# Hi-PACE/hipace

Measured on AMD Instinct MI355X. Metric: transverse slices/s at 1024^2 x 4ppc (explicit solver), higher is better.
Workload: dtype f64

## Files before the change

### hipace_amd/_lib.py

```python
import ctypes as C
import os
import subprocess


def hip_already_started():
    import sys
    if _LIB is not None:
        return True
    t = sys.modules.get("torch")
    try:
        return bool(t is not None and t.cuda.is_initialized())
    except Exception:
        return False


_LIB = None
_HWQ_PRESET = "GPU_MAX_HW_QUEUES" in os.environ
_HIP_STARTED_AT_IMPORT = hip_already_started()
_HERE = os.path.dirname(os.path.abspath(__file__))
CSRC = os.path.join(_HERE, "csrc")
SO = os.environ.get("HPS_LIB") or os.path.join(CSRC, "libhpslice.so")


class Slab(C.Structure):
# ... 115 lines not shown
                                           C.c_int, C.c_int, C.c_void_p, C.c_void_p, C.c_void_p]),
    "hps_deposit_current_tiled_laser": (C.c_int, [Slab, Plasma, Geom, C.c_void_p, C.c_int, C.c_double, C.c_double, C.c_int,
                                                  C.c_double, C.c_int, C.c_void_p, C.c_void_p, C.c_void_p, C.c_void_p]),
    "hps_explicit_deposit_tiled_laser": (C.c_int, [Slab, Plasma, Geom, C.c_void_p, C.c_int, C.c_void_p, C.c_double, C.c_double,
                                                   C.c_int, C.c_int, C.c_int, C.c_void_p, C.c_void_p, C.c_void_p]),
    "hps_advance_plasma_tiled_laser": (C.c_int, [Slab, Plasma, Geom, C.c_void_p, C.c_int, C.c_double, C.c_double, C.c_int,
                                                 C.c_int, C.c_int, C.c_int, C.c_void_p, C.c_void_p, C.c_void_p]),
    "hps_tiling_set_validity": (C.c_int, [C.c_void_p, C.c_int, C.c_int]),
    "hps_particles_record": (C.c_int, [C.c_int]),
    "hps_particles_recorded": (C.c_int, [C.c_char_p, C.c_long, C.POINTER(C.c_long)]),
    "hps_poisson_create": (C.c_int, [C.c_int, C.c_int, C.c_double, C.c_double, C.POINTER(C.c_void_p)]),
    "hps_poisson_solve": (C.c_int, [C.c_void_p, C.c_void_p, Slab, C.c_int, C.c_void_p]),
    "hps_poisson_solve_batch": (C.c_int, [C.c_void_p, C.c_int, C.c_void_p, Slab, C.c_void_p, C.c_void_p]),
    "hps_poisson_info": (C.c_int, [C.c_void_p, C.POINTER(C.c_int), C.POINTER(C.c_int), C.POINTER(C.c_int)]),
    "hps_poisson_destroy": (C.c_int, [C.c_void_p]),
    "hps_mg_create": (C.c_int, [C.c_int, C.c_int, C.c_double, C.c_double, C.POINTER(C.c_void_p)]),
    "hps_mg_solve1": (C.c_int, [C.c_void_p, Slab, C.c_int, C.c_int, C.c_int, C.c_double, C.c_double, C.c_int,
                                C.POINTER(C.c_int), C.POINTER(C.c_double), C.c_void_p]),
    "hps_mg_solve1_fabs": (C.c_int, [C.c_void_p, Slab, Slab, Slab, C.c_double, C.c_double, C.c_int,
                                     C.POINTER(C.c_int), C.POINTER(C.c_double), C.c_void_p]),
    "hps_mg_info": (C.c_int, [C.c_void_p, C.POINTER(C.c_int), C.POINTER(C.c_int), C.POINTER(C.c_int), C.POINTER(C.c_int),
                              C.POINTER(C.c_long), C.POINTER(C.c_int), C.POINTER(C.c_int), C.POINTER(C.c_int), C.POINTER(C.c_int)]),
    "hps_mg_info_schedule": (C.c_int, [C.c_void_p, C.POINTER(C.c_int)]),
    "hps_mg_destroy": (C.c_int, [C.c_void_p]),
    "hps_mg2_create": (C.c_int, [C.c_int, C.c_int, C.c_double, C.c_double, C.POINTER(C.c_void_p)]),
    "hps_mg2_solve2": (C.c_int, [C.c_void_p, C.c_void_p, C.c_void_p, C.c_void_p, C.c_void_p, C.c_double, C.c_double, C.c_int,
                                 C.POINTER(C.c_int), C.POINTER(C.c_double), C.c_void_p]),
    "hps_mg2_info": (C.c_int, [C.c_void_p, C.POINTER(C.c_int), C.POINTER(C.c_int), C.POINTER(C.c_int), C.POINTER(C.c_int)]),
    "hps_mg2_destroy": (C.c_int, [C.c_void_p]),
    "hps_engine_laser_vcycles": (C.c_int, [C.c_void_p, C.POINTER(C.c_long)]),
    "hps_engine_create": (C.c_int, [C.POINTER(Deck), C.c_int, C.POINTER(C.c_void_p)]),
    "hps_engine_destroy": (C.c_int, [C.c_void_p]),
    "hps_engine_begin_step": (C.c_int, [C.c_void_p]),
    "hps_engine_solve_slice": (C.c_int, [C.c_void_p, C.c_int]),
    "hps_engine_solve_slice_begin": (C.c_int, [C.c_void_p, C.c_int]),
    "hps_engine_solve_slice_finish": (C.c_int, [C.c_void_p, C.c_int]),
    "hps_engine_slice_ready": (C.c_int, [C.c_void_p]),
    "hps_engine_run_step": (C.c_int, [C.c_void_p]),
    "hps_engine_sync": (C.c_int, [C.c_void_p]),
    "hps_engine_info": (C.c_int, [C.c_void_p, C.POINTER(C.c_int), C.POINTER(C.c_int), C.POINTER(C.c_long)]),
    "hps_engine_slab": (Slab, [C.c_void_p]),
    "hps_engine_plasma": (Plasma, [C.c_void_p]),
    "hps_engine_stream": (C.c_void_p, [C.c_void_p]),
    "hps_engine_ions": (Plasma, [C.c_void_p]),
    "hps_engine_ion_stats": (C.c_int, [C.c_void_p, C.POINTER(C.c_long), C.POINTER(C.c_long)]),
    "hps_engine_checksums": (C.c_int, [C.c_void_p, C.c_void_p]),
# ... 193 lines not shown
```

### hipace_amd/api.py

```python
import ctypes as C

import numpy as np
import torch

from . import _lib, decks as _decks, expr as _expr
from ._lib import CIDX, COMPS, ID_VALID, PL_REAL, check


def _stream():
    return C.c_void_p(torch.cuda.current_stream().cuda_stream)


def _iarr(vals):
    return (C.c_int * len(vals))(*[int(v) for v in vals])


class Geometry:

    def __init__(self, nx, ny, lo, hi, dz, bc=1, normalized=True, consts=(1., 1., 1., 1., 1.), ng=None):
        self.nx, self.ny = nx, ny
        g = _lib.Geom()
        g.dx = (hi[0] - lo[0]) / nx
        g.dy = (hi[1] - lo[1]) / ny
        g.dz = dz
# ... 321 lines not shown

class MultiGrid:

    def __init__(self, nx, ny, dx, dy):
        self._h = C.c_void_p()
        check(_lib.lib().hps_mg_create(nx, ny, dx, dy, C.byref(self._h)))

    LOWV = ("v3", "v-cc", "v-nodal", "bottom")
    TILES = ("TileSmall", "TileBig", "TileSmall-pull", "TileMid-pull")

    def info(self, schedule=False):
        cc, nl, lb, kind, npyr, nres, pull1 = (C.c_int() for _ in range(7))
        lds, t = C.c_long(), (C.c_int * 31)()
        check(_lib.lib().hps_mg_info(self._h, C.byref(cc), C.byref(nl), C.byref(lb), C.byref(kind), C.byref(lds), t,
                                     C.byref(pull1), C.byref(npyr), C.byref(nres)))
        out = {"cc": bool(cc.value), "nlev": nl.value, "lowv_begin": lb.value, "lowv": self.LOWV[kind.value],
               "lowv_lds": lds.value, "tiles": tuple(self.TILES[v] for v in t if v >= 0), "nodal_pull1": bool(pull1.value),
               "pyramid": npyr.value, "restricts": nres.value}
        if schedule:
            guest = C.c_int()
            check(_lib.lib().hps_mg_info_schedule(self._h, C.byref(guest)))
            out["coef_guest"] = bool(guest.value)
        return out

    def solve1(self, fields, sol_comp, rhs_comp, acoef_comp, tol_rel=1e-4, tol_abs=2.2250738585072014e-308,
               nummaxiter=200):
        it = C.c_int()
        rn = C.c_double()
        check(_lib.lib().hps_mg_solve1(self._h, fields.struct(), sol_comp, rhs_comp, acoef_comp, tol_rel, tol_abs,
                                       nummaxiter, C.byref(it), C.byref(rn), _stream()))
        return it.value, rn.value

    def solve1_fabs(self, sol, rhs, acoef, tol_rel=1e-4, tol_abs=2.2250738585072014e-308, nummaxiter=200):
        it = C.c_int()
        rn = C.c_double()
        check(_lib.lib().hps_mg_solve1_fabs(self._h, sol.struct(), rhs.struct(), acoef.struct(), tol_rel, tol_abs, nummaxiter,
                                            C.byref(it), C.byref(rn), _stream()))
        return it.value, rn.value

    def __del__(self):
        if getattr(self, "_h", None) and _lib is not None:
            _lib.lib().hps_mg_destroy(self._h)
            self._h = None


class Expression:
# ... 910 lines not shown
```

### hipace_amd/csrc/multigrid.hip

```cpp
#include "common.h"
#include <type_traits>
#include "mg_gate.h"
#include "slab_ops.h"

#include <vector>
#include <algorithm>
#include <cmath>
#include <cstring>

namespace hps {

struct FView {
    double* p; long js, ns; int oi, oj;
    __device__ __forceinline__ double& operator() (int i, int j, int n) const {
        const unsigned o = (unsigned)((i + oi) + (j + oj)*(int)js + n*(int)ns)*8u;
        return *reinterpret_cast<double*>(reinterpret_cast<char*>(p) + o);
    }
};

struct LevBox { int lox, loy, hix, hiy;
                int vlx, vly, vhx, vhy; };

enum { SRC_ZERO = 0, SRC_DIRECT = 1, SRC_PROLONG = 2 };

// ... 89 lines not shown
    if (CC) return crse(ic, jc, n);
    const bool io = (i & 1), jo = (j & 1);
    if (io && jo)  return (crse(ic, jc, n) + crse(ic+1, jc, n) + crse(ic, jc+1, n) + crse(ic+1, jc+1, n))*0.25;
    if (io)        return (crse(ic, jc, n) + crse(ic+1, jc, n))*0.5;
    if (jo)        return (crse(ic, jc, n) + crse(ic, jc+1, n))*0.5;
    return crse(ic, jc, n);
}

constexpr int MG_MAX_VCYCLES = 1024;
template <int NT>
__device__ __forceinline__ void block_max_to (unsigned long long* slot, double v, double* s_red)
{
    for (int o = 32; o > 0; o >>= 1) v = fmax(v, __shfl_xor(v, o));
    if ((threadIdx.x & 63) == 0) s_red[threadIdx.x >> 6] = v;
    __syncthreads();
    if (threadIdx.x == 0) {
        double m = 0.0;
        for (int w = 0; w < NT/64; ++w) m = fmax(m, s_red[w]);
        if (m > 0.0) atomicMax(slot + (blockIdx.x & (MG_NSUB - 1)), (unsigned long long)__double_as_longlong(m));
    }
    __syncthreads();
}

#define MG_ROWPK(m) const int jj = BR ? (tid / PR)*GPAIRS + (m) : (tid + MG_NT*(m)) / PR, pk = BR ? (tid & (PR - 1)) : (tid + MG_NT*(m)) - jj*PR
template <bool CC> __device__ __forceinline__ double restrict_at (const FView& fine, int i, int j, int n);
template <class TS, bool CC, int SRC, bool DO_RES, bool FUSE_R, bool INTERIOR, int NSW, bool GATE_IN = (NSW == 4), bool RPULL = false>
__device__ __forceinline__ void smooth_tile (double (&s_phi)[2][TS::AY*TS::AX], double* s_red, double* s_crs, const LevBox& b, const FView& phi_out,
                                             const FView& phi_out2, const FView& rhs, const FView& acf, const FView& phi_in, const FView& crse,
                                             const FView& res_out, const FView& cres_out, double facx, double facy,
                                             int gi0, int gj0, unsigned long long* resnorm, unsigned long long* rhsnorm, const StopRule& sr)
{
    constexpr int E = DO_RES ? NSW : NSW - 1;
    constexpr int GT_X = TS::TX, GT_Y = TS::TY, GA_X = TS::AX, GA_Y = TS::AY, MG_NT = TS::NT, GPAIRS = TS::GPAIRS, PR = TS::PR;
    constexpr int AXH = GA_X/2, CH = GA_Y*AXH;
    constexpr bool BR = GPAIRS <= 2 || INTERIOR;
    const int tid = threadIdx.x;
    const int cpar = (gi0 + gj0) & 1;
    MG_STAMP(0);
    double r0[GPAIRS][2], r1[GPAIRS][2], ac[GPAIRS][2], ci[GPAIRS][2];
    bool in[GPAIRS][2];
    int hx[GPAIRS];
    double fxm[GPAIRS][2], fym[GPAIRS];
    double rmax = 0.0;
#pragma unroll
    for (int m = 0; m < GPAIRS; ++m) {
        MG_ROWPK(m);
// ... 101 lines not shown

    double l0[GPAIRS][2], l1[GPAIRS][2];
    if constexpr (BR) {
#pragma unroll
        for (int m = 0; m < GPAIRS; ++m) {
            MG_ROWPK(m);
            const int row = (jj + 1)*AXH + pk;
#pragma unroll
            for (int p = 0; p < 2; ++p) { const int h = hx[m] ^ p; l0[m][p] = s_phi[0][p*CH + row + h]; l1[m][p] = s_phi[1][p*CH + row + h]; }
        }
#pragma unroll
        for (int icolor = 0; icolor < NSW; ++icolor) {
            const int p = icolor & 1;
#pragma unroll
            for (int m = 0; m < GPAIRS; ++m) {
                MG_ROWPK(m);
                const int h = hx[m] ^ p;
                const int row = (jj + 1)*AXH + pk;
                const double* nb0 = &s_phi[0][(1 - p)*CH + row];
                const double* nb1 = &s_phi[1][(1 - p)*CH + row];
                const double we0 = nb0[h] + l0[m][1 - p], we1 = nb1[h] + l1[m][1 - p];
                const double s0 = (m > 0) ? l0[m > 0 ? m - 1 : 0][1 - p] : nb0[h - AXH], s1 = (m > 0) ? l1[m > 0 ? m - 1 : 0][1 - p] : nb1[h - AXH];
                const double t0 = (m + 1 < GPAIRS) ? l0[m + 1 < GPAIRS ? m + 1 : m][1 - p] : nb0[h + AXH], t1 = (m + 1 < GPAIRS) ? l1[m + 1 < GPAIRS ? m + 1 : m][1 - p] : nb1[h + AXH];
                const double n0 = (r0[m][p] - (fxm[m][p]*we0 + fym[m]*(s0 + t0)))*ci[m][p];
                const double n1 = (r1[m][p] - (fxm[m][p]*we1 + fym[m]*(s1 + t1)))*ci[m][p];
                if (INTERIOR || in[m][p]) { s_phi[0][p*CH + row + h] = n0; s_phi[1][p*CH + row + h] = n1; l0[m][p] = n0; l1[m][p] = n1; }
            }
            __syncthreads();
        }
    } else {
#pragma unroll
        for (int icolor = 0; icolor < NSW; ++icolor) {
            constexpr int dummy = 0; (void)dummy;
            const int p = icolor & 1;
#pragma unroll
            for (int m = 0; m < GPAIRS; ++m) {
                MG_ROWPK(m);
                const int h = hx[m] ^ p;
                const int row = (jj + 1)*AXH + pk;
                const double* nb0 = &s_phi[0][(1 - p)*CH + row];
                const double* nb1 = &s_phi[1][(1 - p)*CH + row];
                const double n0 = (r0[m][p] - (fxm[m][p]*(nb0[0] + nb0[1]) + fym[m]*(nb0[h - AXH] + nb0[h + AXH])))*ci[m][p];
                const double n1 = (r1[m][p] - (fxm[m][p]*(nb1[0] + nb1[1]) + fym[m]*(nb1[h - AXH] + nb1[h + AXH])))*ci[m][p];
                if (INTERIOR || in[m][p]) { s_phi[0][p*CH + row + h] = n0; s_phi[1][p*CH + row + h] = n1; }
            }
            __syncthreads();
        }
    }
    MG_STAMP(3);

    double resmax = 0.0;
    if constexpr (BR) {
        double la0[GPAIRS], ra0[GPAIRS], la1[GPAIRS], ra1[GPAIRS];
        bool finr[GPAIRS];
#pragma unroll
        for (int m = 0; m < GPAIRS; ++m) {
            MG_ROWPK(m);
            const int j = gj0 + jj;
            const bool rowok = (jj >= E && jj < GT_Y - E);
            double q0[2], q1[2];
            bool fin[2];
#pragma unroll
            for (int p = 0; p < 2; ++p) {
                const int h = hx[m] ^ p;
                const int ii = 2*pk + h;
                fin[p] = rowok && ii >= E && ii < GT_X - E && in[m][p];
// ... 115 lines not shown
    if constexpr (HOST > 0) {
        static_assert(2*TS::AY*TS::AX >= COEF_GUEST_MAX_IMG, "the image is staged in the tile's static LDS");
        if (blockIdx.x == 0) { coef_guest_derive(&s_phi[0][0], guest..., TS::NT); return; }
    }
    constexpr bool PLDS = !CC && SRC == SRC_PROLONG;
    __shared__ double s_crs[PLDS ? 2*(TS::AX/2 + 2)*(TS::AY/2 + 2) : 1];
    constexpr int E = DO_RES ? NSW : NSW - 1;
    constexpr int FX = GT_X - 2*E, FY = GT_Y - 2*E;
    const unsigned wg = blockIdx.x - HOST;
    const int nb = gridDim.x - HOST, q8 = nb >> 3, r8 = nb & 7, xcd = wg & 7;
    const int tile = xcd*q8 + min(xcd, r8) + (wg >> 3);
    const int bx = tile % ntx, by = tile / ntx;
    const int gi0 = b.vlx + bx*FX - E;
    const int gj0 = b.vly + by*FY - E;
    const bool interior = (gi0 - 1 >= b.vlx) && (gi0 + GT_X <= b.vhx) && (gj0 - 1 >= b.vly) && (gj0 + GT_Y <= b.vhy)
                       && (gi0 > b.lox) && (gi0 + GT_X - 1 < b.hix) && (gj0 > b.loy) && (gj0 + GT_Y - 1 < b.hiy);
    constexpr bool GATE_IN = (NSW == 4);
    if (interior) smooth_tile<TS, CC, SRC, DO_RES, FUSE_R, true, NSW, GATE_IN, RPULL>(s_phi, s_red, s_crs, b, phi_out, phi_out2, rhs, acf, phi_in, crse, res_out, cres_out,
                                                             facx, facy, gi0, gj0, resnorm, rhsnorm, sr);
    else          smooth_tile<TS, CC, SRC, DO_RES, FUSE_R, false, NSW, GATE_IN, RPULL>(s_phi, s_red, s_crs, b, phi_out, phi_out2, rhs, acf, phi_in, crse, res_out, cres_out,
                                                              facx, facy, gi0, gj0, resnorm, rhsnorm, sr);
}

template <bool CC>
__device__ __forceinline__ double restrict_at (const FView& fine, int i, int j, int n)
{
    if (CC) return 0.25*(fine(2*i, 2*j, n) + fine(2*i+1, 2*j, n) + fine(2*i, 2*j+1, n) + fine(2*i+1, 2*j+1, n));
    return (1./16.)*(fine(2*i-1, 2*j-1, n) + 2.*fine(2*i, 2*j-1, n) + fine(2*i+1, 2*j-1, n)
                   + 2.*fine(2*i-1, 2*j, n) + 4.*fine(2*i, 2*j, n) + 2.*fine(2*i+1, 2*j, n)
                   + fine(2*i-1, 2*j+1, n) + 2.*fine(2*i, 2*j+1, n) + fine(2*i+1, 2*j+1, n));
}

template <bool CC>
__global__ __launch_bounds__(256)
void k_restrict (LevBox cb, FView crse, FView fine, int ncomp, StopRule sr)
{
    if (!vcycle_active(sr)) return;
    const int i = cb.vlx + blockIdx.x*blockDim.x + threadIdx.x;
    const int j = cb.vly + blockIdx.y;
    if (i > cb.vhx || j > cb.vhy) return;
    for (int n = 0; n < ncomp; ++n) crse(i, j, n) = restrict_at<CC>(fine, i, j, n);
}

typedef __attribute__((address_space(3))) double lds_double;

struct LowLev { LevBox b; int nxb; int cells; int off; };
// ... 833 lines not shown

struct Multigrid {
    bool cc; int nx, ny; double dx, dy;
    bool hierarchy_ready = false;
    bool nodal_pull1 = false;
    std::vector<MGLevelDev> L;
    int lowv_begin = 1;
    LowLev* d_low = nullptr; size_t low_lds = 0;
    bool bottom = false;
    unsigned long long *d_buf = nullptr, *h_buf = nullptr;
    unsigned long long* h_buf_dev = nullptr;
    long dbg_trips = 0, dbg_solves = 0, dbg_hist[8] = {0,0,0,0,0,0,0,0};
    unsigned long long* h_seq = nullptr; unsigned long long* h_seq_dev = nullptr; unsigned long long seq = 0;
    unsigned long long* d_norms = nullptr;
    unsigned long long* h_norms = nullptr;
    int last_iters = 1;
    SolveRun run{};
    bool defer_post = false; bool deferred_valid = false; MgPost deferred{};
    bool use_low3 = false; Low2 low3{}; Low2* d_low3 = nullptr; size_t low3_lds = 0;
    bool ride_on = false; ShiftInit ride{}; int ride_guests = 0;
    double* cinvA = nullptr;
    double* coef_img = nullptr;
    bool coef_guest = false;
    double* tmp0 = nullptr;
    bool cor_in_tmp = false;
    FView sol, rhs, acf0;

    ~Multigrid () {
        for (auto& l : L) { (void)hipFree(l.acf); (void)hipFree(l.res); (void)hipFree(l.cor); (void)hipFree(l.rescor); }
        if (getenv("HPS_MG_DEBUG")) fprintf(stderr, "mg: solves %ld trips %ld hist %ld %ld %ld %ld %ld %ld\n", dbg_solves, dbg_trips, dbg_hist[0], dbg_hist[1], dbg_hist[2], dbg_hist[3], dbg_hist[4], dbg_hist[5]);
        (void)hipFree(d_buf); (void)hipFree(d_low); (void)hipFree(tmp0); (void)hipFree(d_low3); (void)hipFree(cinvA); (void)hipFree(coef_img);
        if (h_buf) (void)hipHostFree(h_buf);
    }
    FView lv (int il, double* p) const {
        const MGLevelDev& l = L[il];
        const long nxb = l.b.hix - l.b.lox + 1;
        return FView{p, nxb, l.cells, -l.b.lox, -l.b.loy};
    }
    int nlev () const { return (int)L.size(); }
    bool pulls (int il) const {
        return !cc && ((il >= 2 && ((il < lowv_begin && L[il].cells <= SMALL_TILE_CELLS) ||
                                    (il == lowv_begin && !use_low3 && !bottom))) ||
                       (il == 1 && nodal_pull1));
    }
};

// ... 67 lines not shown
            M->low3_lds = (size_t)off3*sizeof(double);
            if (M->low3_lds > 64*1024)
                HPS_HIP_CHECK(hipFuncSetAttribute((const void*)k_lower_v3, hipFuncAttributeMaxDynamicSharedMemorySize, (int)M->low3_lds));
            HPS_HIP_CHECK(hipMalloc(&M->d_low3, sizeof(Low2)));
            HPS_HIP_CHECK(hipMemcpy(M->d_low3, &e, sizeof(Low2), hipMemcpyHostToDevice));
            HPS_HIP_CHECK(hipMalloc(&M->cinvA, (size_t)e.nx[0]*e.ny[0]*sizeof(double)));
            int dev = 0, ncu = 0;
            HPS_HIP_CHECK(hipGetDevice(&dev));
            HPS_HIP_CHECK(hipDeviceGetAttribute(&ncu, hipDeviceAttributeMultiprocessorCount, dev));
            M->ride_guests = std::max(ncu - 2, 1);
            const char* sw = getenv("HPS_MG_COEF_GUEST");
            M->coef_guest = !(sw && atoi(sw) == 0) && M->L[0].cells > SMALL_TILE_CELLS && e.nl > 1 && e.ctot <= COEF_GUEST_MAX_IMG;
            break;
        }
    }
    if (!M->use_low3) {
        long cells = 0;
        for (int il = M->lowv_begin; il < nl; ++il) cells += M->L[il].cells;
        M->low_lds = (size_t)(8*cells)*sizeof(double);
        hipFuncAttributes fa{};
        HPS_HIP_CHECK(hipFuncGetAttributes(&fa, M->cc ? (const void*)k_lower_v<true> : (const void*)k_lower_v<false>));
        if (M->low_lds + fa.sharedSizeBytes > device_max_lds()) { M->bottom = true; M->lowv_begin = nl - 1; M->low_lds = 0; }
    }
    M->nodal_pull1 = !M->cc && M->lowv_begin > 1;
    if (!M->use_low3 && !M->bottom) {
        std::vector<LowLev> low;
        int off = 0;
        for (int il = M->lowv_begin; il < nl; ++il) {
            const MGLevelDev& l = M->L[il];
            low.push_back(LowLev{l.b, l.b.hix - l.b.lox + 1, (int)l.cells, off});
            off += 8*(int)l.cells;
        }
        if (M->low_lds > 64*1024) {
            HPS_HIP_CHECK(hipFuncSetAttribute((const void*)k_lower_v<true>, hipFuncAttributeMaxDynamicSharedMemorySize, (int)M->low_lds));
            HPS_HIP_CHECK(hipFuncSetAttribute((const void*)k_lower_v<false>, hipFuncAttributeMaxDynamicSharedMemorySize, (int)M->low_lds));
        }
        HPS_HIP_CHECK(hipMalloc(&M->d_low, low.size()*sizeof(LowLev)));
        HPS_HIP_CHECK(hipMemcpy(M->d_low, low.data(), low.size()*sizeof(LowLev), hipMemcpyHostToDevice));
    }
    HPS_HIP_CHECK(hipMalloc(&M->d_buf, (3 + MG_MAX_VCYCLES)*MG_NSUB*sizeof(unsigned long long)));
    HPS_HIP_CHECK(hipHostMalloc(&M->h_buf, ((3 + MG_MAX_VCYCLES)*MG_NSUB + 8)*sizeof(unsigned long long), hipHostMallocMapped));
    HPS_HIP_CHECK(hipHostGetDevicePointer((void**)&M->h_buf_dev, M->h_buf, 0));
    M->h_seq = M->h_buf + (3 + MG_MAX_VCYCLES)*MG_NSUB; M->h_seq_dev = M->h_buf_dev + (3 + MG_MAX_VCYCLES)*MG_NSUB;
    *M->h_seq = 0ULL;
    HPS_HIP_CHECK(hipMemset(M->d_buf, 0, (3 + MG_MAX_VCYCLES)*MG_NSUB*sizeof(unsigned long long)));
    memset(M->h_buf, 0, (3 + MG_MAX_VCYCLES)*MG_NSUB*sizeof(unsigned long long));
// ... 10 lines not shown
                              const StopRule& sr, hipStream_t st)
{
    const LevBox& b = M->L[il].b;
    constexpr int E = DO_RES ? NSW : NSW - 1;
    constexpr int FX = TS::TX - 2*E, FY = TS::TY - 2*E;
    const int ntx = ceil_div(b.vhx - b.vlx + 1, FX), nty = ceil_div(b.vhy - b.vly + 1, FY);
    const double fac = (double)(1 << il);
    const double ldx = M->dx*fac, ldy = M->dy*fac;
    const double facx = 1.0/(ldx*ldx), facy = 1.0/(ldy*ldy);
    constexpr bool FUSE = CC && DO_RES;
    hipLaunchKernelGGL((k_smooth<TS, CC, SRC, DO_RES, FUSE, NSW, RPULL>), dim3(ntx*nty), dim3(TS::NT), 0, st, b, phi_out, phi_out2, rhs, acf,
                       phi_in, crse, res_out, cres_out, facx, facy, ntx, resnorm, rhsnorm, sr);
}

template <bool CC, int SRC, bool DO_RES>
static void launch_smooth (Multigrid* M, int il, FView phi_out, FView phi_out2, FView rhs, FView acf, FView phi_in, FView crse,
                           FView res_out, FView cres_out, unsigned long long* resnorm, unsigned long long* rhsnorm,
                           const StopRule& sr, hipStream_t st)
{
    if (M->L[il].cells <= SMALL_TILE_CELLS)
        launch_smooth_ts<TileSmall, CC, SRC, DO_RES>(M, il, phi_out, phi_out2, rhs, acf, phi_in, crse, res_out, cres_out, resnorm, rhsnorm, sr, st);
    else
        launch_smooth_ts<TileBig, CC, SRC, DO_RES>(M, il, phi_out, phi_out2, rhs, acf, phi_in, crse, res_out, cres_out, resnorm, rhsnorm, sr, st);
}

template <bool CC>
static void restrict_residual_if_nodal (Multigrid* M, int il, const StopRule& sr, hipStream_t st)
{
    if (CC) return;
    const LevBox& cb = M->L[il+1].b;
    hipLaunchKernelGGL(k_restrict<CC>, dim3(ceil_div(cb.vhx - cb.vlx + 1, 64), cb.vhy - cb.vly + 1), dim3(64), 0, st,
                       cb, M->lv(il+1, M->L[il+1].res), M->lv(il, M->L[il].rescor), 2, sr);
}

template <bool CC>
static void vcycle (Multigrid* M, int k, double tol_rel, double tol_abs, hipStream_t st)
{
    const int nl = M->nlev();
    const int lb = M->lowv_begin;
    const FView none{};
    const StopRule sr{M->d_norms, k, tol_rel, tol_abs};
    for (int il = 1; il < lb; ++il) {
        if (!M->pulls(il))
            launch_smooth<CC, SRC_ZERO, true>(M, il, M->lv(il, M->L[il].cor), none, M->lv(il, M->L[il].res), M->lv(il, M->L[il].acf), none,
                                              none, M->lv(il, M->L[il].rescor), M->lv(il+1, M->L[il+1].res), nullptr, nullptr, sr, st);
        else if constexpr (!CC) {
// ... 6 lines not shown
        }
        if (!M->pulls(il + 1)) restrict_residual_if_nodal<CC>(M, il, sr, st);
    }
    {
        const double fac = (double)(1 << lb);
        const double ldx = M->dx*fac, ldy = M->dy*fac;
        const LevBox& bb = M->L[nl-1].b;
        const int nsweeps = std::max(16, (std::max(bb.hix - bb.lox + 1, bb.hiy - bb.loy + 1) + 1)/2*2);
        if (M->bottom) {
            const FView cor = M->lv(lb, M->L[lb].cor), rhs = M->lv(lb, M->L[lb].res), acf = M->lv(lb, M->L[lb].acf);
            const dim3 grid(ceil_div(bb.vhx - bb.vlx + 1, 64), bb.vhy - bb.vly + 1);
            for (int is = -1; is < nsweeps; ++is)
                hipLaunchKernelGGL(k_bottom_sweep<CC>, grid, dim3(64), 0, st, bb, cor, rhs, acf, 1.0/(ldx*ldx), 1.0/(ldy*ldy), is, sr);
        } else if (M->use_low3) {
            const int guests = (k == 0 && M->ride_on) ? M->ride_guests : 0;
            M->ride_on = false;
            hipLaunchKernelGGL(k_lower_v3, dim3(2 + guests), dim3(1024), M->low3_lds, st, M->d_low3, M->L[lb].acf, M->cinvA, M->L[lb].res, M->L[lb].cor,
                               M->coef_img, M->low3.nx[0], M->low3.ny[0], M->low3.ctot, 1.0/(ldx*ldx), 1.0/(ldy*ldy), nsweeps, sr, M->ride,
                               M->coef_guest ? 0 : 1);
        } else
            hipLaunchKernelGGL(k_lower_v<CC>, dim3(CC ? 1 : 2), dim3(1024), M->low_lds, st, M->d_low, nl - lb, M->L[lb].acf, M->L[lb].res,
                               M->L[lb].cor, 1.0/(ldx*ldx), 1.0/(ldy*ldy), nsweeps, sr, M->pulls(lb) ? M->lv(lb-1, M->L[lb-1].rescor) : FView{});
    }
    for (int il = lb - 1; il >= 1; --il) {
        double* crse = (il + 1 == lb) ? M->L[il+1].cor : M->L[il+1].rescor;
        launch_smooth<CC, SRC_PROLONG, false>(M, il, M->lv(il, M->L[il].rescor), none, M->lv(il, M->L[il].res), M->lv(il, M->L[il].acf),
                                              M->lv(il, M->L[il].cor), M->lv(il+1, crse), none, none, nullptr, nullptr, sr, st);
    }
    {
        double* crse = (1 == lb) ? M->L[1].cor : M->L[1].rescor;
        double* in = M->cor_in_tmp ? M->tmp0 : M->L[0].cor;
        double* out = M->cor_in_tmp ? M->L[0].cor : M->tmp0;
        launch_smooth_ts<typename HugeTileOf<CC>::type, CC, SRC_PROLONG, true, 8>(M, 0, M->lv(0, out), M->sol, M->rhs, M->acf0, M->lv(0, in), M->lv(1, crse),
                                                             M->lv(0, M->L[0].rescor), M->lv(1, M->L[1].res), M->d_norms + (2 + k)*MG_NSUB,
                                                             nullptr, sr, st);
        M->cor_in_tmp = !M->cor_in_tmp;
    }
    if (!M->nodal_pull1) restrict_residual_if_nodal<CC>(M, 0, sr, st);
}

__global__ __launch_bounds__(256)
void k_post_norms (const unsigned long long* __restrict__ src, volatile unsigned long long* dst, int nwords,
                   volatile unsigned long long* seq_slot, unsigned long long seq, int* go_word, StopRule after)
{
    {   const bool act = vcycle_active(after);
        if (threadIdx.x == 0) *go_word = act ? 0 : 1; }
    for (int w = threadIdx.x; w < nwords; w += blockDim.x) dst[w] = src[w];
    HPS_HOST_STORES_ACKNOWLEDGED();
    __syncthreads();
    if (threadIdx.x == 0) { *seq_slot = seq; }
}
// ... 287 lines not shown
    if (tiles) {
        for (int il = 0; il < HPS_MG_MAXLEV; ++il) {
            int t = -1;
            if (il < lb) {
                const bool small = M->L[il].cells <= SMALL_TILE_CELLS;
                t = M->pulls(il) ? (small ? HPS_MG_TILE_SMALL_PULL : HPS_MG_TILE_MID_PULL) : (small ? HPS_MG_TILE_SMALL : HPS_MG_TILE_BIG);
            }
            tiles[il] = t;
        }
    }
    if (nodal_pull1) *nodal_pull1 = M->nodal_pull1;
    if (pyr_levels) *pyr_levels = std::min(lb, M->cc ? 5 : NPYR_MAX);
    if (pyr_restricts) *pyr_restricts = lb - std::min(lb, M->cc ? 5 : NPYR_MAX);
    return HPS_OK;
}

extern "C" int hps_mg_info_schedule (void* handle, int* coef_guest)
{
    HPS_REQUIRE(handle, "hps_mg_info_schedule: null handle");
    if (coef_guest) *coef_guest = static_cast<const Multigrid*>(handle)->coef_guest ? 1 : 0;
    return HPS_OK;
}

extern "C" int hps_mg_solve1 (void* handle, hps_slab slab, int sol_comp, int rhs_comp, int acoef_comp, double tol_rel,
                              double tol_abs, int max_iters, int* iters_host, double* resnorm_host, hps_stream stream)
{
    HPS_REQUIRE(handle && slab.p, "hps_mg_solve1: null argument");
    Multigrid* M = static_cast<Multigrid*>(handle);
    HPS_REQUIRE(slab.nx == M->nx && slab.ny == M->ny, "hps_mg_solve1: slab size does not match the solver");
    HPS_REQUIRE(sol_comp >= 0 && sol_comp + 1 < slab.ncomp && rhs_comp >= 0 && rhs_comp + 1 < slab.ncomp &&
                acoef_comp >= 0 && acoef_comp < slab.ncomp, "hps_mg_solve1: bad component");
    HPS_REQUIRE(M->cc || slab.ng >= 1, "hps_mg_solve1: node-centred solve needs >= 1 guard cell");
    HPS_REQUIRE(slab.nstride < (1L << 27) && slab.ng <= 8, "hps_mg_solve1: planes of at most 2^27 doubles and at most 8 guard cells (32-bit byte offsets in the kernels)");
    return mg_solve1(M, slab, sol_comp, rhs_comp, acoef_comp, tol_rel, tol_abs, max_iters, iters_host, resnorm_host,
                     (hipStream_t)stream);
}

extern "C" int hps_mg_solve1_fabs (void* handle, hps_slab sol2, hps_slab rhs2, hps_slab acoef1, double tol_rel, double tol_abs,
                                   int max_iters, int* iters_host, double* resnorm_host, hps_stream stream)
{
    HPS_REQUIRE(handle && sol2.p && rhs2.p && acoef1.p, "hps_mg_solve1_fabs: null argument");
    Multigrid* M = static_cast<Multigrid*>(handle);
    for (const hps_slab* s : {&sol2, &rhs2, &acoef1}) {
        HPS_REQUIRE(s->nx == M->nx && s->ny == M->ny, "hps_mg_solve1_fabs: view size does not match the solver");
        HPS_REQUIRE(M->cc || s->ng >= 1, "hps_mg_solve1_fabs: node-centred solve needs >= 1 guard cell in every view");
    }
// ... 42 lines not shown
```

### include/hpslice.h

```cpp
#ifndef HPSLICE_H_
#define HPSLICE_H_

#include <stdint.h>

#ifdef __cplusplus
extern "C" {
#endif

typedef void* hps_stream;

enum { HPS_OK = 0, HPS_ERR_ARG = 1, HPS_ERR_HIP = 2, HPS_ERR_FFT = 3, HPS_ERR_MG_DIVERGED = 4,
       HPS_ERR_MG_MAXITER = 5, HPS_ERR_COMM = 6, HPS_ERR_UNSUPPORTED = 7 };

enum { HPS_BC_REFLECTING = 0, HPS_BC_PERIODIC = 1, HPS_BC_ABSORBING = 2 };

typedef struct {
    double* p;
    int nx, ny, ng, ncomp;
    long jstride, nstride;
} hps_slab;

typedef struct {
    double *x, *y, *w, *ux, *uy, *psi, *x_prev, *y_prev, *ux_half, *uy_half, *psi_half;
    uint64_t* idcpu;
// ... 79 lines not shown


int hps_poisson_create (int nx, int ny, double dx, double dy, void** handle);
int hps_poisson_solve (void* handle, const double* staging, hps_slab dst, int dst_comp,
                       hps_stream stream);
int hps_poisson_solve_batch (void* handle, int nbatch, const double* staging, hps_slab dst,
                             const int* dst_comps, hps_stream stream);
enum { HPS_POISSON_OWN_SYM = 0, HPS_POISSON_OWN_POW2 = 1, HPS_POISSON_DENSE = 2, HPS_POISSON_ROCFFT = 3 };
int hps_poisson_info (void* handle, int* backend, int* x_len, int* tri_rows);
int hps_poisson_destroy (void* handle);

int hps_mg_create (int nx, int ny, double dx, double dy, void** handle);
int hps_mg_solve1 (void* handle, hps_slab slab, int sol_comp, int rhs_comp, int acoef_comp,
                   double tol_rel, double tol_abs, int max_iters, int* iters_host,
                   double* resnorm_host, hps_stream stream);
int hps_mg_solve1_fabs (void* handle, hps_slab sol2, hps_slab rhs2, hps_slab acoef1, double tol_rel, double tol_abs,
                        int max_iters, int* iters_host, double* resnorm_host, hps_stream stream);
enum { HPS_MG_LOWV_V3 = 0, HPS_MG_LOWV_CC = 1, HPS_MG_LOWV_NODAL = 2, HPS_MG_LOWV_BOTTOM = 3 };
enum { HPS_MG_TILE_SMALL = 0, HPS_MG_TILE_BIG = 1, HPS_MG_TILE_SMALL_PULL = 2, HPS_MG_TILE_MID_PULL = 3 };
enum { HPS_MG_MAXLEV = 31 };
int hps_mg_info (void* handle, int* cc, int* nlev, int* lowv_begin, int* lowv_kind, long* lowv_lds, int* tiles,
                 int* nodal_pull1, int* pyr_levels, int* pyr_restricts);
int hps_mg_info_schedule (void* handle, int* coef_guest);
int hps_mg_destroy (void* handle);

int hps_mg2_create (int nx, int ny, double dx, double dy, void** handle);
int hps_mg2_solve2 (void* handle, double* sol2_dev, const double* rhs2_dev, const double* acoef_real_dev,
                    const double* acoef_imag_dev, double tol_rel, double tol_abs, int max_iters, int* iters_host,
                    double* resnorm_host, hps_stream stream);
enum { HPS_MG2_BOTTOM_LOWER_V = 0, HPS_MG2_BOTTOM_SINGLE_BLOCK = 1, HPS_MG2_BOTTOM_PER_SWEEP = 2 };
enum { HPS_MG2_TILE_SINGLE_BLOCK = 0, HPS_MG2_TILE_SMALL = 1, HPS_MG2_TILE_BIG = 2 };
int hps_mg2_info (void* handle, int* nlev, int* low_top, int* bottom, int* tiles);
int hps_mg2_destroy (void* handle);


#define HPS_MAX_ION_LEVELS 56
typedef struct {
    int nx, ny, nz; double lo[3], hi[3];
    int order; int deriv_type;
    int plasma_ppc[2]; double plasma_density; double plasma_radius;
    double plasma_charge, plasma_mass; double max_qsa; int n_subcycles;
    int beam_profile;
    double beam_zmin, beam_zmax, beam_radius, beam_density;
    double beam_umean[3], beam_pos_mean[3], beam_pos_std[3]; int beam_ppc[3]; double beam_charge;
    int bc; double mg_tol_rel, mg_tol_abs; int deposit_rho; int n_steps;
    double dt; int beam_n_subcycles; double beam_mass; double ext_E_slope[2];
// ... 270 lines not shown
```

Before: 1761.

## Fuse multigrid up-leg prolongation-smooth across mid levels into one kernel

Adds a kernel that performs the V-cycle up-leg (prolongation plus Gauss-Seidel sweeps) for two or three consecutive mid levels in a single launch. Each tile recomputes overlapping halos on the coarser levels in shared memory, which removes per-level kernel launches and global round-trips of the corrected fields. The cost is redundant halo work, heavy register and LDS use, and occupancy limited to one block per CU. The GS update is also factored into a helper with explicit FMA and contraction off, keeping rounding consistent between the old and new paths.

```diff
diff --git a/hipace_amd/_lib.py b/hipace_amd/_lib.py
--- a/hipace_amd/_lib.py
+++ b/hipace_amd/_lib.py
@@ -161,6 +161,7 @@
     "hps_mg_info": (C.c_int, [C.c_void_p, C.POINTER(C.c_int), C.POINTER(C.c_int), C.POINTER(C.c_int), C.POINTER(C.c_int),
                               C.POINTER(C.c_long), C.POINTER(C.c_int), C.POINTER(C.c_int), C.POINTER(C.c_int), C.POINTER(C.c_int)]),
     "hps_mg_info_schedule": (C.c_int, [C.c_void_p, C.POINTER(C.c_int)]),
+    "hps_mg_info_upleg": (C.c_int, [C.c_void_p, C.POINTER(C.c_int)]),
     "hps_mg_destroy": (C.c_int, [C.c_void_p]),
     "hps_mg2_create": (C.c_int, [C.c_int, C.c_int, C.c_double, C.c_double, C.POINTER(C.c_void_p)]),
     "hps_mg2_solve2": (C.c_int, [C.c_void_p, C.c_void_p, C.c_void_p, C.c_void_p, C.c_void_p, C.c_double, C.c_double, C.c_int,
diff --git a/hipace_amd/api.py b/hipace_amd/api.py
--- a/hipace_amd/api.py
+++ b/hipace_amd/api.py
@@ -367,6 +367,11 @@
             check(_lib.lib().hps_mg_info_schedule(self._h, C.byref(guest)))
             out["coef_guest"] = bool(guest.value)
         return out
+
+    def upleg_fused_levels(self):
+        n = C.c_int()
+        check(_lib.lib().hps_mg_info_upleg(self._h, C.byref(n)))
+        return n.value
 
     def solve1(self, fields, sol_comp, rhs_comp, acoef_comp, tol_rel=1e-4, tol_abs=2.2250738585072014e-308,
                nummaxiter=200):
diff --git a/hipace_amd/csrc/multigrid.hip b/hipace_amd/csrc/multigrid.hip
--- a/hipace_amd/csrc/multigrid.hip
+++ b/hipace_amd/csrc/multigrid.hip
@@ -135,6 +135,13 @@
     __syncthreads();
 }
 
+__device__ __forceinline__ double gs_cell (double rhs, double fxm, double we, double fym, double s, double n, double ci)
+{
+#pragma clang fp contract(off)
+    const double t = fym*(s + n);
+    return (rhs - __builtin_fma(fxm, we, t))*ci;
+}
+
 #define MG_ROWPK(m) const int jj = BR ? (tid / PR)*GPAIRS + (m) : (tid + MG_NT*(m)) / PR, pk = BR ? (tid & (PR - 1)) : (tid + MG_NT*(m)) - jj*PR
 template <bool CC> __device__ __forceinline__ double restrict_at (const FView& fine, int i, int j, int n);
 template <class TS, bool CC, int SRC, bool DO_RES, bool FUSE_R, bool INTERIOR, int NSW, bool GATE_IN = (NSW == 4), bool RPULL = false>
@@ -282,8 +289,8 @@
                 const double we0 = nb0[h] + l0[m][1 - p], we1 = nb1[h] + l1[m][1 - p];
                 const double s0 = (m > 0) ? l0[m > 0 ? m - 1 : 0][1 - p] : nb0[h - AXH], s1 = (m > 0) ? l1[m > 0 ? m - 1 : 0][1 - p] : nb1[h - AXH];
                 const double t0 = (m + 1 < GPAIRS) ? l0[m + 1 < GPAIRS ? m + 1 : m][1 - p] : nb0[h + AXH], t1 = (m + 1 < GPAIRS) ? l1[m + 1 < GPAIRS ? m + 1 : m][1 - p] : nb1[h + AXH];
-                const double n0 = (r0[m][p] - (fxm[m][p]*we0 + fym[m]*(s0 + t0)))*ci[m][p];
-                const double n1 = (r1[m][p] - (fxm[m][p]*we1 + fym[m]*(s1 + t1)))*ci[m][p];
+                const double n0 = gs_cell(r0[m][p], fxm[m][p], we0, fym[m], s0, t0, ci[m][p]);
+                const double n1 = gs_cell(r1[m][p], fxm[m][p], we1, fym[m], s1, t1, ci[m][p]);
                 if (INTERIOR || in[m][p]) { s_phi[0][p*CH + row + h] = n0; s_phi[1][p*CH + row + h] = n1; l0[m][p] = n0; l1[m][p] = n1; }
             }
             __syncthreads();
@@ -300,8 +307,8 @@
                 const int row = (jj + 1)*AXH + pk;
                 const double* nb0 = &s_phi[0][(1 - p)*CH + row];
                 const double* nb1 = &s_phi[1][(1 - p)*CH + row];
-                const double n0 = (r0[m][p] - (fxm[m][p]*(nb0[0] + nb0[1]) + fym[m]*(nb0[h - AXH] + nb0[h + AXH])))*ci[m][p];
-                const double n1 = (r1[m][p] - (fxm[m][p]*(nb1[0] + nb1[1]) + fym[m]*(nb1[h - AXH] + nb1[h + AXH])))*ci[m][p];
+                const double n0 = gs_cell(r0[m][p], fxm[m][p], nb0[0] + nb0[1], fym[m], nb0[h - AXH], nb0[h + AXH], ci[m][p]);
+                const double n1 = gs_cell(r1[m][p], fxm[m][p], nb1[0] + nb1[1], fym[m], nb1[h - AXH], nb1[h + AXH], ci[m][p]);
                 if (INTERIOR || in[m][p]) { s_phi[0][p*CH + row + h] = n0; s_phi[1][p*CH + row + h] = n1; }
             }
             __syncthreads();
@@ -463,6 +470,205 @@
                                                               facx, facy, gi0, gj0, resnorm, rhsnorm, sr);
 }
 
+struct UpLevArg { LevBox b; FView rhs, acf, cor; double facx, facy; };
+struct UpArgs { UpLevArg l[3]; FView crse, out; int ntx; };
+
+template <int SX_, int SY_, int NT_, bool INTERIOR, bool GCRSE>
+struct UpLev {
+    static constexpr int SX = SX_, SY = SY_, NT = NT_, AX = SX + 2, AY = SY + 2, AXH = AX/2, CH = AY*AXH, PR = SX/2;
+    static constexpr int GP = (PR*SY + NT - 1)/NT;
+    static constexpr int NF = (AX*AY + NT - 1)/NT;
+    static constexpr int NBLK = SY/GP;
+    static_assert(SX % 2 == 0 && SY % GP == 0 && PR*NBLK <= NT, "level shape");
+    int gi0, gj0, cpar, pk, blk;
+    double r0[GP][2], r1[GP][2], ac[GP][2], ci[GP][2], fxm[GP][2], fym[GP];
+    bool in[GP][2];
+    int hx[GP];
+    double v0[NF], v1[NF], c0[GCRSE ? NF : 1], c1[GCRSE ? NF : 1];
+    double l0[GP][2], l1[GP][2];
+
+    __device__ __forceinline__ void issue (const UpLevArg& a, const FView& crse, int gi0_, int gj0_)
+    {
+        const LevBox& b = a.b;
+        const int tid = threadIdx.x;
+        gi0 = gi0_; gj0 = gj0_; cpar = (gi0 + gj0) & 1;
+        const bool live = tid < PR*NBLK;
+        blk = live ? tid / PR : 0; pk = tid % PR;
+#pragma unroll
+        for (int m = 0; m < GP; ++m) {
+            const int j = gj0 + blk*GP + m;
+            hx[m] = (gi0 + 2*pk + j) & 1;
+#pragma unroll
+            for (int p = 0; p < 2; ++p) {
+                const int i = gi0 + 2*pk + (hx[m] ^ p);
+                const int ic = INTERIOR ? i : min(max(i, b.vlx), b.vhx), jc = INTERIOR ? j : min(max(j, b.vly), b.vhy);
+                in[m][p] = live && (INTERIOR || (ic == i && jc == j));
+                r0[m][p] = a.rhs(ic, jc, 0); r1[m][p] = a.rhs(ic, jc, 1); ac[m][p] = a.acf(ic, jc, 0);
+            }
+        }
+#pragma unroll
+        for (int m = 0; m < NF; ++m) {
+            const int s = min(tid + NT*m, AX*AY - 1);
+            const int lj = s / AX, li = s - lj*AX;
+            const int i = gi0 - 1 + li, j = gj0 - 1 + lj;
+            const int ic = INTERIOR ? i : min(max(i, b.vlx), b.vhx), jc = INTERIOR ? j : min(max(j, b.vly), b.vhy);
+            v0[m] = a.cor(ic, jc, 0); v1[m] = a.cor(ic, jc, 1);
+            if constexpr (GCRSE) { c0[m] = crse(ic >> 1, jc >> 1, 0); c1[m] = crse(ic >> 1, jc >> 1, 1); }
+        }
+    }
+    __device__ __forceinline__ void keep () const
+    {
+#pragma unroll
+        for (int m = 0; m < GP; ++m) { HPS_KEEP(r0[m][0]); HPS_KEEP(r0[m][1]); HPS_KEEP(r1[m][0]); HPS_KEEP(r1[m][1]); HPS_KEEP(ac[m][0]); HPS_KEEP(ac[m][1]); }
+#pragma unroll
+        for (int m = 0; m < NF; ++m) { HPS_KEEP(v0[m]); HPS_KEEP(v1[m]); if constexpr (GCRSE) { HPS_KEEP(c0[m]); HPS_KEEP(c1[m]); } }
+    }
+    __device__ __forceinline__ void coefficients (const UpLevArg& a)
+    {
+        const LevBox& b = a.b;
+#pragma unroll
+        for (int m = 0; m < GP; ++m) {
+            const int j = gj0 + blk*GP + m;
+            fym[m] = INTERIOR ? a.facy : wall_mult<true>(j, b.loy, b.hiy, a.facy);
+#pragma unroll
+            for (int p = 0; p < 2; ++p) {
+                const int i = gi0 + 2*pk + (hx[m] ^ p);
+                fxm[m][p] = INTERIOR ? a.facx : wall_mult<true>(i, b.lox, b.hix, a.facx);
+                const bool ok = in[m][p];
+                r0[m][p] = ok ? r0[m][p] : 0.0;
+                r1[m][p] = ok ? r1[m][p] : 0.0;
+                ac[m][p] = ok ? ac[m][p] : 0.0;
+                ci[m][p] = 1.0/diag_c0<true>(i, j, b, ac[m][p], a.facx, a.facy);
+            }
+        }
+    }
+    template <class CL>
+    __device__ __forceinline__ void fill (double* s, const UpLevArg& a, const CL* cl, const double* sc)
+    {
+        const LevBox& b = a.b;
+        const int tid = threadIdx.x;
+#pragma unroll
+        for (int m = 0; m < NF; ++m) {
+            const int q = tid + NT*m;
+            if (q < AX*AY) {
+                const int lj = q / AX, li = q - lj*AX;
+                const int i = gi0 - 1 + li, j = gj0 - 1 + lj;
+                const int ic = INTERIOR ? i : min(max(i, b.vlx), b.vhx), jc = INTERIOR ? j : min(max(j, b.vly), b.vhy);
+                double a0 = v0[m], a1 = v1[m];
+                if constexpr (GCRSE) { a0 += c0[m]; a1 += c1[m]; }
+                else {
+                    const int cli = (ic >> 1) - (cl->gi0 - 1), clj = (jc >> 1) - (cl->gj0 - 1);
+                    const int oc = ((cl->cpar + cli + clj) & 1)*CL::CH + clj*CL::AXH + (cli >> 1);
+                    a0 += sc[oc]; a1 += sc[2*CL::CH + oc];
+                }
+                const bool inside = INTERIOR || (ic == i && jc == j);
+                const int o = ((cpar + li + lj) & 1)*CH + lj*AXH + (li >> 1);
+                s[o] = inside ? a0 : 0.0; s[2*CH + o] = inside ? a1 : 0.0;
+            }
+        }
+    }
+    __device__ __forceinline__ void sweeps (double* s)
+    {
+        double* s0p = s; double* s1p = s + 2*CH;
+#pragma unroll
+        for (int m = 0; m < GP; ++m) {
+            const int row = (blk*GP + m + 1)*AXH + pk;
+#pragma unroll
+            for (int p = 0; p < 2; ++p) { const int h = hx[m] ^ p; l0[m][p] = s0p[p*CH + row + h]; l1[m][p] = s1p[p*CH + row + h]; }
+        }
+#pragma unroll
+        for (int icolor = 0; icolor < 4; ++icolor) {
+            const int p = icolor & 1;
+#pragma unroll
+            for (int m = 0; m < GP; ++m) {
+                const int h = hx[m] ^ p;
+                const int row = (blk*GP + m + 1)*AXH + pk;
+                const double* nb0 = &s0p[(1 - p)*CH + row];
+                const double* nb1 = &s1p[(1 - p)*CH + row];
+                const double we0 = nb0[h] + l0[m][1 - p], we1 = nb1[h] + l1[m][1 - p];
+                const double b0 = (m > 0) ? l0[m > 0 ? m - 1 : 0][1 - p] : nb0[h - AXH], b1 = (m > 0) ? l1[m > 0 ? m - 1 : 0][1 - p] : nb1[h - AXH];
+                const double t0 = (m + 1 < GP) ? l0[m + 1 < GP ? m + 1 : m][1 - p] : nb0[h + AXH], t1 = (m + 1 < GP) ? l1[m + 1 < GP ? m + 1 : m][1 - p] : nb1[h + AXH];
+                const double n0 = gs_cell(r0[m][p], fxm[m][p], we0, fym[m], b0, t0, ci[m][p]);
+                const double n1 = gs_cell(r1[m][p], fxm[m][p], we1, fym[m], b1, t1, ci[m][p]);
+                if (INTERIOR || in[m][p]) { s0p[p*CH + row + h] = n0; s1p[p*CH + row + h] = n1; l0[m][p] = n0; l1[m][p] = n1; }
+            }
+            __syncthreads();
+        }
+    }
+    __device__ __forceinline__ void store (const FView& out) const
+    {
+#pragma unroll
+        for (int m = 0; m < GP; ++m) {
+            const int jj = blk*GP + m;
+            const bool rowok = (jj >= 3 && jj < SY - 3);
+#pragma unroll
+            for (int p = 0; p < 2; ++p) {
+                const int ii = 2*pk + (hx[m] ^ p);
+                if (rowok && ii >= 3 && ii < SX - 3 && in[m][p]) { out(gi0 + ii, gj0 + jj, 0) = l0[m][p]; out(gi0 + ii, gj0 + jj, 1) = l1[m][p]; }
+            }
+        }
+    }
+};
+
+__device__ __forceinline__ int up_coarse_origin (int g, int vl, int vh) { return (min(max(g - 1, vl), vh) >> 1) - 3; }
+
+template <class TS, int NL, bool INTERIOR>
+__device__ __forceinline__ void up_fused_tile (double* s1, double* s2, double* s3, const UpArgs& A, int gi0, int gj0, const StopRule& sr)
+{
+    constexpr int X2 = (TS::TX + 2)/2 + 7, Y2 = (TS::TY + 2)/2 + 7, X3 = (X2 + 2)/2 + 7, Y3 = (Y2 + 2)/2 + 7;
+    UpLev<TS::TX, TS::TY, TS::NT, INTERIOR, false> L1;
+    UpLev<X2, Y2, TS::NT, false, NL == 2> L2;
+    UpLev<X3, Y3, TS::NT, false, true> L3;
+    const int g2i = up_coarse_origin(gi0, A.l[0].b.vlx, A.l[0].b.vhx), g2j = up_coarse_origin(gj0, A.l[0].b.vly, A.l[0].b.vhy);
+    L1.issue(A.l[0], A.crse, gi0, gj0);
+    L2.issue(A.l[1], A.crse, g2i, g2j);
+    if constexpr (NL == 3)
+        L3.issue(A.l[2], A.crse, up_coarse_origin(g2i, A.l[1].b.vlx, A.l[1].b.vhx), up_coarse_origin(g2j, A.l[1].b.vly, A.l[1].b.vhy));
+    {
+        const bool active = vcycle_active(sr);
+        L1.keep(); L2.keep();
+        if constexpr (NL == 3) L3.keep();
+        if (!active) return;
+    }
+    if constexpr (NL == 3) {
+        L3.coefficients(A.l[2]);
+        L3.fill(s3, A.l[2], &L3, s3);
+        __syncthreads();
+        L3.sweeps(s3);
+    }
+    L2.coefficients(A.l[1]);
+    L2.fill(s2, A.l[1], &L3, s3);
+    __syncthreads();
+    L2.sweeps(s2);
+    L1.coefficients(A.l[0]);
+    L1.fill(s1, A.l[0], &L2, s2);
+    __syncthreads();
+    L1.sweeps(s1);
+    L1.store(A.out);
+}
+
+template <class TS, int NL>
+__global__ __launch_bounds__(TS::NT, 1)
+void k_up_fused (UpArgs A, StopRule sr)
+{
+    static_assert(NL == 2 || NL == 3, "two or three mid levels");
+    constexpr int X2 = (TS::TX + 2)/2 + 7, Y2 = (TS::TY + 2)/2 + 7, X3 = (X2 + 2)/2 + 7, Y3 = (Y2 + 2)/2 + 7;
+    __shared__ double s1[2*TS::AX*TS::AY];
+    __shared__ double s2[2*(X2 + 2)*(Y2 + 2)];
+    __shared__ double s3[NL == 3 ? 2*(X3 + 2)*(Y3 + 2) : 1];
+    constexpr int E = 3, FX = TS::TX - 2*E, FY = TS::TY - 2*E;
+    const LevBox& b = A.l[0].b;
+    const unsigned wg = blockIdx.x;
+    const int nb = gridDim.x, q8 = nb >> 3, r8 = nb & 7, xcd = wg & 7;
+    const int tile = xcd*q8 + min(xcd, r8) + (wg >> 3);
+    const int bx = tile % A.ntx, by = tile / A.ntx;
+    const int gi0 = b.vlx + bx*FX - E, gj0 = b.vly + by*FY - E;
+    const bool interior = (gi0 - 1 >= b.vlx) && (gi0 + TS::TX <= b.vhx) && (gj0 - 1 >= b.vly) && (gj0 + TS::TY <= b.vhy)
+                       && (gi0 > b.lox) && (gi0 + TS::TX - 1 < b.hix) && (gj0 > b.loy) && (gj0 + TS::TY - 1 < b.hiy);
+    if (interior) up_fused_tile<TS, NL, true>(s1, s2, s3, A, gi0, gj0, sr);
+    else          up_fused_tile<TS, NL, false>(s1, s2, s3, A, gi0, gj0, sr);
+}
+
 template <bool CC>
 __device__ __forceinline__ double restrict_at (const FView& fine, int i, int j, int n)
 {
@@ -1342,6 +1548,7 @@
     double* cinvA = nullptr;
     double* coef_img = nullptr;
     bool coef_guest = false;
+    int up_fused = 0;
     double* tmp0 = nullptr;
     bool cor_in_tmp = false;
     FView sol, rhs, acf0;
@@ -1455,6 +1662,10 @@
         HPS_HIP_CHECK(hipFuncGetAttributes(&fa, M->cc ? (const void*)k_lower_v<true> : (const void*)k_lower_v<false>));
         if (M->low_lds + fa.sharedSizeBytes > device_max_lds()) { M->bottom = true; M->lowv_begin = nl - 1; M->low_lds = 0; }
     }
+    {
+        const char* sw = getenv("HPS_MG_UP_FUSED");
+        if (!(sw && atoi(sw) == 0) && M->cc && M->use_low3 && M->lowv_begin >= 3) M->up_fused = std::min(3, M->lowv_begin - 1);
+    }
     M->nodal_pull1 = !M->cc && M->lowv_begin > 1;
     if (!M->use_low3 && !M->bottom) {
         std::vector<LowLev> low;
@@ -1511,6 +1722,32 @@
         launch_smooth_ts<TileSmall, CC, SRC, DO_RES>(M, il, phi_out, phi_out2, rhs, acf, phi_in, crse, res_out, cres_out, resnorm, rhsnorm, sr, st);
     else
         launch_smooth_ts<TileBig, CC, SRC, DO_RES>(M, il, phi_out, phi_out2, rhs, acf, phi_in, crse, res_out, cres_out, resnorm, rhsnorm, sr, st);
+}
+
+template <class TS, int NL>
+static void launch_up_fused_ts (Multigrid* M, int lb, const StopRule& sr, hipStream_t st)
+{
+    UpArgs A{};
+    for (int k = 0; k < NL; ++k) {
+        const int il = 1 + k;
+        const double fac = (double)(1 << il);
+        const double ldx = M->dx*fac, ldy = M->dy*fac;
+        A.l[k] = UpLevArg{M->L[il].b, M->lv(il, M->L[il].res), M->lv(il, M->L[il].acf), M->lv(il, M->L[il].cor), 1.0/(ldx*ldx), 1.0/(ldy*ldy)};
+    }
+    A.crse = M->lv(NL + 1, (NL + 1 == lb) ? M->L[NL+1].cor : M->L[NL+1].rescor);
+    A.out = M->lv(1, M->L[1].rescor);
+    const LevBox& b = M->L[1].b;
+    constexpr int FX = TS::TX - 6, FY = TS::TY - 6;
+    const int ntx = ceil_div(b.vhx - b.vlx + 1, FX), nty = ceil_div(b.vhy - b.vly + 1, FY);
+    A.ntx = ntx;
+    hipLaunchKernelGGL((k_up_fused<TS, NL>), dim3(ntx*nty), dim3(TS::NT), 0, st, A, sr);
+}
+
+static void launch_up_fused (Multigrid* M, int lb, const StopRule& sr, hipStream_t st)
+{
+    const bool small = M->L[1].cells <= SMALL_TILE_CELLS;
+    if (M->up_fused == 3) { if (small) launch_up_fused_ts<TileSmall, 3>(M, lb, sr, st); else launch_up_fused_ts<TileBig, 3>(M, lb, sr, st); }
+    else                  { if (small) launch_up_fused_ts<TileSmall, 2>(M, lb, sr, st); else launch_up_fused_ts<TileBig, 2>(M, lb, sr, st); }
 }
 
 template <bool CC>
@@ -1563,11 +1800,12 @@
             hipLaunchKernelGGL(k_lower_v<CC>, dim3(CC ? 1 : 2), dim3(1024), M->low_lds, st, M->d_low, nl - lb, M->L[lb].acf, M->L[lb].res,
                                M->L[lb].cor, 1.0/(ldx*ldx), 1.0/(ldy*ldy), nsweeps, sr, M->pulls(lb) ? M->lv(lb-1, M->L[lb-1].rescor) : FView{});
     }
-    for (int il = lb - 1; il >= 1; --il) {
+    for (int il = lb - 1; il > (CC ? M->up_fused : 0); --il) {
         double* crse = (il + 1 == lb) ? M->L[il+1].cor : M->L[il+1].rescor;
         launch_smooth<CC, SRC_PROLONG, false>(M, il, M->lv(il, M->L[il].rescor), none, M->lv(il, M->L[il].res), M->lv(il, M->L[il].acf),
                                               M->lv(il, M->L[il].cor), M->lv(il+1, crse), none, none, nullptr, nullptr, sr, st);
     }
+    if constexpr (CC) if (M->up_fused) launch_up_fused(M, lb, sr, st);
     {
         double* crse = (1 == lb) ? M->L[1].cor : M->L[1].rescor;
         double* in = M->cor_in_tmp ? M->tmp0 : M->L[0].cor;
@@ -1901,6 +2139,13 @@
     return HPS_OK;
 }
 
+extern "C" int hps_mg_info_upleg (void* handle, int* fused_levels)
+{
+    HPS_REQUIRE(handle, "hps_mg_info_upleg: null handle");
+    if (fused_levels) *fused_levels = static_cast<const Multigrid*>(handle)->up_fused;
+    return HPS_OK;
+}
+
 extern "C" int hps_mg_solve1 (void* handle, hps_slab slab, int sol_comp, int rhs_comp, int acoef_comp, double tol_rel,
                               double tol_abs, int max_iters, int* iters_host, double* resnorm_host, hps_stream stream)
 {
diff --git a/include/hpslice.h b/include/hpslice.h
--- a/include/hpslice.h
+++ b/include/hpslice.h
@@ -125,6 +125,7 @@
 int hps_mg_info (void* handle, int* cc, int* nlev, int* lowv_begin, int* lowv_kind, long* lowv_lds, int* tiles,
                  int* nodal_pull1, int* pyr_levels, int* pyr_restricts);
 int hps_mg_info_schedule (void* handle, int* coef_guest);
+int hps_mg_info_upleg (void* handle, int* fused_levels);
 int hps_mg_destroy (void* handle);
 
 int hps_mg2_create (int nx, int ny, double dx, double dy, void** handle);
```

Result: faster. 1788 (median of 6 runs) (+1.5%).
